# Ichoran/dbce-video-cpp

Measured on AMD Instinct MI355X. Metric: frames/s + raw-pixel GB/s, 4096x3072 U8 encode+decode round-trip, higher is better.
Workload: dtype u8

## Files before the change

### dbde-video-cpp_amd/csrc/dbde_kernels.hip

```cpp
#include "dbde_kernels.h"

#include "dbde_bits.h"
#include "dbde_device.h"


namespace dbde {

#ifndef DBDE_DIAG_LATE
#define DBDE_DIAG_LATE 34
#endif
#ifdef DBDE_DIAG
#define SF_DECL uint64_t sfd[10] = {0, 0, 0, 0, 0, 0, 0, 0, 0, 0}
#define SF_MARK(i) do { if (threadIdx.x == 0) sfd[i] = wall_clock64(); } while (0)
#define SF_DRAIN() asm volatile("s_waitcnt vmcnt(0) lgkmcnt(0)" ::: "memory")
#define SF_FLUSH(diag, last)                                                                          \
    do {                                                                                              \
        if (threadIdx.x == 0 && (diag)) {                                                             \
            atomicMax(&(diag)[0], ~(unsigned long long)sfd[0]);                                       \
            for (int i_ = 1; i_ < 10; i_++) atomicAdd(&(diag)[i_], (unsigned long long)sfd[i_]);      \
            atomicAdd(&(diag)[10], 1ull);                                                             \
            atomicMax(&(diag)[11], (unsigned long long)sfd[last]);                                    \
            atomicMax(&(diag)[12], (unsigned long long)sfd[0]);                                       \
            atomicAdd(&(diag)[13], (unsigned long long)sfd[0]);                                       \
        }                                                                                             \
// ... 1463 lines not shown
    const uint32_t seg = (cpf + blockDim.x - 1u) / blockDim.x;
    const uint32_t k0 = (uint32_t)tid * seg;
    uint32_t local = 0;
    for (uint32_t k = k0; k < k0 + seg && k < cpf; k++) local += s_sum[k];
    uint32_t incl = local;
#pragma unroll
    for (int o = 1; o < 64; o <<= 1) {
        uint32_t n = __shfl_up(incl, o, 64);
        if (lane >= o) incl += n;
    }
    if (lane == 63) s_part[wave] = incl;
    __syncthreads();
    uint32_t base = 0, total = 0;
    for (int k = 0; k < (int)(blockDim.x >> 6); k++) {
        const uint32_t v = s_part[k];
        if (k < wave) base += v;
        total += v;
    }
    uint32_t run = base + incl - local;
    uint32_t *co = p.chunk_off + (size_t)f * (cpf + 1u);
    for (uint32_t k = k0; k < k0 + seg && k < cpf; k++) {
        co[k] = run;
        run += s_sum[k];
    }
    if (tid == 0) co[cpf] = total;

    if (tid == 0) {
        bool ok = in_range;
        uint32_t field = 0;
        uint64_t index = 0, elapsed = 0, consumed = 20;
        if (in_extent(off, 20, p.stream_bytes)) {
            field = load_u32_bytes(fb);
            index = load_u64_bytes(fb + 4);
            elapsed = f64_to_u64_x86(__longlong_as_double((long long)load_u64_bytes(fb + 12)));
        }
        if (ok) {
            const int32_t nb = (int32_t)load_u32_bytes(fb + 20);
            const int32_t nm = (int32_t)load_u32_bytes(fb + 24 + T);
            const int32_t n64 = (int32_t)load_u32_bytes(fb + 28 + meta_t);
            ok = nb == (int32_t)T && nm == (int32_t)(T * p.min_bytes) && n64 == (int32_t)total && !(s_flags & 1u);
            if (ok && !in_extent(off, need + 8ull * total, p.stream_bytes)) ok = false;
            if (ok) consumed = need + 8ull * total;
        }
        p.frame_ok[f] = ok ? 1u : 0u;
        if (p.results) {
            FrameResultDev *r = reinterpret_cast<FrameResultDev *>(p.results) + f;
            r->u64s = (field == 2u && ok) ? 2u : 0xFFFFFFFFu;
            r->pad_ = 0;
            r->index = index;
            r->elapsed_ns = elapsed;
            r->consumed = consumed;
        }
    }
}

__global__ __launch_bounds__(256) void decode_index_split_kernel(IdxParams p) {
    __shared__ uint32_t s_part[4];
    __shared__ uint32_t s_last;

    const uint32_t f = blockIdx.x / p.split, piece = blockIdx.x - f * p.split;
    const int tid = threadIdx.x, lane = tid & 63, wave = tid >> 6;
    const uint32_t T = p.T, cpf = p.chunks_per_frame;
    const uint64_t off = p.frame_offsets[f];
    const uint64_t meta_t = (1ull + p.min_bytes) * T;
    const uint64_t need = 32ull + meta_t;
    const bool in_range = in_extent(off, need, p.stream_bytes);
    const uint8_t *fb = p.stream + off;
    uint32_t *co = p.chunk_off + (size_t)f * (cpf + 1u);

    const uint32_t per = (cpf + p.split - 1u) / p.split;
    const uint32_t k_begin = piece * per, k_end = k_begin + per < cpf ? k_begin + per : cpf;
    uint32_t bad = 0;
    for (uint32_t k = k_begin + (uint32_t)wave; k < k_end; k += 4u) {
        uint32_t sum = 0;
        if (in_range) {
            const uint8_t *darr = fb + 24;
            const uint32_t c_lo = dec_chunk_begin(p.geom, k), c_hi = dec_chunk_begin(p.geom, k + 1u);
#pragma unroll
            for (uint32_t j = 0; j < 8u; j += 4u) {
                const uint32_t q = c_lo + (uint32_t)lane * 8u + j;
                if (q < c_hi) {
                    uint32_t x;
                    __builtin_memcpy(&x, darr + q, 4);
                    const uint32_t keep = c_hi - q;
                    if (keep < 4u) x &= 0xFFFFFFFFu >> (8u * (4u - keep));
                    bad |= depth_bytes_bad(x, p.min_bytes);
                    sum += __builtin_amdgcn_sad_u8(x, 0u, 0u);
                }
            }
        }
        const uint32_t tot = wave_scan_incl(sum);
        if (lane == 63) __hip_atomic_store(&co[k], tot, __ATOMIC_RELAXED, __HIP_MEMORY_SCOPE_AGENT);
    }
    if (__any((int)(bad != 0u)) && lane == 0) atomicOr(&p.frame_flag[f], 1u);

    asm volatile("s_waitcnt vmcnt(0)" ::: "memory");
    __syncthreads();
    if (tid == 0) s_last = atomicAdd(&p.frame_ctr[f], 1u) == p.split - 1u ? 1u : 0u;
    __syncthreads();
    if (!s_last) return;

    const uint32_t seg = (cpf + 255u) / 256u;
    const uint32_t k0 = (uint32_t)tid * seg;
    uint32_t local = 0;
    for (uint32_t k = k0; k < k0 + seg && k < cpf; k++)
        local += __hip_atomic_load(&co[k], __ATOMIC_RELAXED, __HIP_MEMORY_SCOPE_AGENT);
    const uint32_t incl = wave_scan_incl(local);
    if (lane == 63) s_part[wave] = incl;
    __syncthreads();
    uint32_t base = 0, total = 0;
#pragma unroll
    for (int k = 0; k < 4; k++) {
        const uint32_t v = s_part[k];
        base += k < wave ? v : 0u;
        total += v;
    }
    uint32_t run = base + incl - local;
    for (uint32_t k = k0; k < k0 + seg && k < cpf; k++) {
        const uint32_t v = __hip_atomic_load(&co[k], __ATOMIC_RELAXED, __HIP_MEMORY_SCOPE_AGENT);
        co[k] = run;
        run += v;
    }
    if (tid == 0) {
        co[cpf] = total;
        const uint32_t flags = __hip_atomic_load(&p.frame_flag[f], __ATOMIC_RELAXED, __HIP_MEMORY_SCOPE_AGENT);
        p.frame_flag[f] = 0;
        p.frame_ctr[f] = 0;
        bool ok = in_range;
        uint32_t field = 0;
        uint64_t index = 0, elapsed = 0, consumed = 20;
        if (in_extent(off, 20, p.stream_bytes)) {
            field = load_u32_bytes(fb);
            index = load_u64_bytes(fb + 4);
            elapsed = f64_to_u64_x86(__longlong_as_double((long long)load_u64_bytes(fb + 12)));
        }
        if (ok) {
            const int32_t nb = (int32_t)load_u32_bytes(fb + 20);
            const int32_t nm = (int32_t)load_u32_bytes(fb + 24 + T);
            const int32_t n64 = (int32_t)load_u32_bytes(fb + 28 + meta_t);
            ok = nb == (int32_t)T && nm == (int32_t)(T * p.min_bytes) && n64 == (int32_t)total && !(flags & 1u);
            if (ok && !in_extent(off, need + 8ull * total, p.stream_bytes)) ok = false;
            if (ok) consumed = need + 8ull * total;
        }
        p.frame_ok[f] = ok ? 1u : 0u;
        if (p.results) {
            FrameResultDev *r = reinterpret_cast<FrameResultDev *>(p.results) + f;
            r->u64s = (field == 2u && ok) ? 2u : 0xFFFFFFFFu;
            r->pad_ = 0;
            r->index = index;
            r->elapsed_ns = elapsed;
            r->consumed = consumed;
        }
    }
}

hipError_t launch_decode_index(const IdxParams &p, int n_frames, hipStream_t s) {
    const size_t lds = (size_t)p.chunks_per_frame * sizeof(uint32_t);
    if (lds > 48 * 1024) {
        hipError_t e = hipFuncSetAttribute(reinterpret_cast<const void *>(decode_index_kernel),
                                           hipFuncAttributeMaxDynamicSharedMemorySize, (int)lds);
        if (e != hipSuccess) return e;
    }
    if (p.split > 1u) {
        hipLaunchKernelGGL(decode_index_split_kernel, dim3((uint32_t)n_frames * p.split), dim3(256), 0, s, p);
        return hipGetLastError();
    }
    const uint32_t pieces = (p.T + 15u) / 16u + 1u;
    uint32_t threads = (pieces + 63u) / 64u * 64u;
    threads = threads < 64u ? 64u : (threads > 1024u ? 1024u : threads);
    hipLaunchKernelGGL(decode_index_kernel, dim3(n_frames), dim3(threads), lds, s, p);
    return hipGetLastError();
}

__device__ __forceinline__ uint32_t swz_byte16(uint32_t A) { return A ^ ((A >> 4) & 0xF0u); }

__device__ __forceinline__ void put_byte1(uint32_t &x, uint32_t sh, uint32_t g) {
    asm("v_lshrrev_b32_sdwa %0, %1, %2 dst_sel:BYTE_1 dst_unused:UNUSED_PRESERVE src0_sel:DWORD src1_sel:DWORD" : "+v"(x) : "v"(sh), "v"(g));
}
__device__ __forceinline__ void put_byte2(uint32_t &x, uint32_t sh, uint32_t g) {
    asm("v_lshrrev_b32_sdwa %0, %1, %2 dst_sel:BYTE_2 dst_unused:UNUSED_PRESERVE src0_sel:DWORD src1_sel:DWORD" : "+v"(x) : "v"(sh), "v"(g));
}
__device__ __forceinline__ void put_byte3(uint32_t &x, uint32_t sh, uint32_t g) {
    asm("v_lshrrev_b32_sdwa %0, %1, %2 dst_sel:BYTE_3 dst_unused:UNUSED_PRESERVE src0_sel:DWORD src1_sel:DWORD" : "+v"(x) : "v"(sh), "v"(g));
}

template <bool SWZ>
__device__ __forceinline__ void unpack_tile_from_lds(const uint8_t *s_img, uint32_t byte_base, uint32_t d,
                                                     uint32_t mn, uint32_t (&v)[16]) {
    const uint32_t mn4 = mn * 0x01010101u;
    const bool d8 = d >= 8u;
    uint32_t a = byte_base;
    const uint32_t md = ((1u << d) - 1u) * 0x01010101u;
    const uint32_t md7 = md & 0x7F7F7F7Fu, mdh = md & 0x80808080u;
    const uint32_t mnlo = mn4 & 0x7F7F7F7Fu, mnhi = mn4 & 0x80808080u;
    const uint32_t d2 = 2u * d, d3 = 3u * d;
#pragma unroll
    for (int r = 0; r < 8; r++) {
        uint32_t t0, t1, t2;
        if (SWZ) {
            const uint32_t A0 = a & ~7u;
            const uint2 lo = *reinterpret_cast<const uint2 *>(s_img + swz_byte16(A0));
            const uint2 hi = *reinterpret_cast<const uint2 *>(s_img + swz_byte16(A0 + 8u));
            const bool up = (a & 4u) != 0u;
            t0 = up ? lo.y : lo.x; t1 = up ? hi.x : lo.y; t2 = up ? hi.y : hi.x;
        } else {
            const uint32_t *q = reinterpret_cast<const uint32_t *>(s_img + (a & ~3u));
            t0 = q[0]; t1 = q[1]; t2 = q[2];
        }
        const uint32_t r_lo = __builtin_amdgcn_alignbyte(t1, t0, a);
        const uint32_t r_hi = __builtin_amdgcn_alignbyte(t2, t1, a);
        const uint32_t g_hi = d8 ? r_hi : __builtin_amdgcn_alignbit(r_hi, r_lo, 4u * d);
        uint32_t x = r_lo, y = g_hi;
        put_byte1(x, d, r_lo); put_byte2(x, d2, r_lo); put_byte3(x, d3, r_lo);
        put_byte1(y, d, g_hi); put_byte2(y, d2, g_hi); put_byte3(y, d3, g_hi);
        v[2 * r] = (((x & md7) + mnlo) ^ (x & mdh)) ^ mnhi;
        v[2 * r + 1] = (((y & md7) + mnlo) ^ (y & mdh)) ^ mnhi;
        a += d;
    }
}

__device__ __forceinline__ void unpack_tile_d8_from_lds(const uint8_t *s_img, uint32_t byte_base, uint32_t mn,
                                                        uint32_t (&v)[16]) {
    const uint32_t mn4 = mn * 0x01010101u;
#pragma unroll
    for (int r = 0; r < 8; r++) {
        const uint2 q = *reinterpret_cast<const uint2 *>(s_img + swz_byte16(byte_base + 8u * (uint32_t)r));
        v[2 * r] = add_bytes(q.x, mn4);
        v[2 * r + 1] = add_bytes(q.y, mn4);
    }
}

constexpr uint32_t kXcdRun = 16;
__device__ __forceinline__ uint32_t xcd_local_chunk(uint32_t b, uint32_t n_chunks) {
    constexpr uint32_t kGroup = 8u * kXcdRun;
    const uint32_t grp = b / kGroup, rem = b % kGroup;
    if ((grp + 1u) * kGroup > n_chunks) return b;
    return grp * kGroup + (rem & 7u) * kXcdRun + (rem >> 3);
}

template <int THREADS = 256>
struct DecLds {
    static constexpr int kThreads = THREADS;
    static constexpr int kWaves = THREADS / 64;
    static constexpr uint32_t kSlots = THREADS == 256 ? 2128u : 1600u;
    static constexpr int kPieces = (kSlots + kThreads - 1) / kThreads;
};

__device__ __forceinline__ void lds_store_u64_any(uint8_t *s_base, uint32_t byte_addr, uint32_t lo, uint32_t hi) {
    const uint64_t v = ((uint64_t)hi << 32) | lo;
    const uint32_t a = (uint32_t)(uintptr_t)(__attribute__((address_space(3))) uint8_t *)s_base + byte_addr;
    asm volatile("ds_write_b64 %0, %1" ::"v"(a), "v"(v) : "memory");
}
__device__ __forceinline__ void lds_store_bytes(uint8_t *s_px, uint32_t a, uint64_t v, uint32_t n) {
    if (n & 4u) { __builtin_memcpy(s_px + a, &v, 4); a += 4u; v >>= 32; }
    if (n & 2u) { s_px[a] = (uint8_t)v; s_px[a + 1u] = (uint8_t)(v >> 8); a += 2u; v >>= 16; }
    if (n & 1u) s_px[a] = (uint8_t)v;
}

__device__ __forceinline__ void store_tile_generic(uint8_t *img, int W, int H, uint32_t w, uint32_t t,
                                                   const uint32_t (&v)[16]) {
    uint32_t ty = t / w, tx = t - ty * w;
    int x0 = 8 * (int)tx;
    int rm = W - x0 < 8 ? W - x0 : 8;
#pragma unroll
    for (int r = 0; r < 8; r++) {
        int yy = 8 * (int)ty + r;
        if (yy < H) {
            uint8_t *row = img + (size_t)yy * (size_t)W + x0;
            const uint64_t q = ((uint64_t)v[2 * r + 1] << 32) | v[2 * r];
            if (rm == 8) {
                store_u64_any(row, q);
            } else {
#pragma unroll
                for (int k = 0; k < 8; k++)
                    if (k < rm) row[k] = (uint8_t)(q >> (8 * k));
            }
        }
    }
}

constexpr int kImgDirect = 0, kImgLinear = 1, kImgTiles = 2;

constexpr int kIdxTable = 0, kIdxSelf = 1, kIdxFused = 2;

template <int IMG, int INDEX, int THREADS = 256>
__global__ __launch_bounds__(THREADS) void decode_kernel(DecParams p) {
    constexpr bool SELF_INDEX = INDEX == kIdxSelf;
    typedef DecLds<THREADS> G;
    __shared__ __attribute__((aligned(16))) uint64_t s_in[G::kSlots * 2];
    __shared__ uint32_t s_wave_tot[G::kWaves];
    __shared__ uint32_t s_idx[G::kWaves][4];

    const int tid = threadIdx.x, lane = tid & 63, wave = tid >> 6;
    SF_DECL;
    SF_MARK(0);
    const uint32_t c = SELF_INDEX ? blockIdx.x : xcd_local_chunk(blockIdx.x, p.n_chunks);
    const uint32_t f = c / p.chunks_per_frame;
    const uint32_t cf = c - f * p.chunks_per_frame;
    const uint64_t foff = p.frame_offsets[f];
    const uint8_t *fb = p.stream + foff;
    const uint32_t t_begin = dec_chunk_begin(p.geom, cf);
    const uint32_t n_tiles = dec_chunk_begin(p.geom, cf + 1u) - t_begin;
    uint32_t w_begin, w_end;
    if (SELF_INDEX) {
        const uint32_t T = p.T;
        const uint64_t need = 32ull + 2ull * T;
        const bool in_range = in_extent(foff, need, p.stream_bytes);
        uint32_t s_before = 0, s_mine = 0, s_all = 0, bad = 0;
        if (in_range) {
            const uint8_t *darr = fb + 24;
            const uint32_t head = (uint32_t)(reinterpret_cast<uintptr_t>(darr) & 15u);
            const uint8_t *a_lo = darr - head;
            const uint32_t npieces = (head + T + 15u) >> 4;
            const uint8_t *s_end = p.stream + p.stream_bytes;
            auto account = [&](uint32_t i, const uint4 &qv) {
                const uint32_t wv[4] = {qv.x, qv.y, qv.z, qv.w};
                const int pos0 = (int)(16u * i) - (int)head;
#pragma unroll
                for (int j = 0; j < 4; j++) {
                    const int pj = pos0 + 4 * j;
                    auto below = [&](int limit) -> uint32_t {
                        const int n = limit - pj;
                        return n >= 4 ? 0xFFFFFFFFu : (n <= 0 ? 0u : (0xFFFFFFFFu >> (8 * (4 - n))));
                    };
                    const uint32_t in = below((int)T) & ~below(0);
                    const uint32_t x = wv[j] & in;
                    bad |= (x & 0xF0F0F0F0u) | ((x + 0x77777777u) & 0x80808080u);
                    const uint32_t m0 = below((int)t_begin), m1 = below((int)(t_begin + n_tiles));
                    s_all += __builtin_amdgcn_sad_u8(x, 0u, 0u);
                    s_before += __builtin_amdgcn_sad_u8(x & m0, 0u, 0u);
                    s_mine += __builtin_amdgcn_sad_u8(x & m1 & ~m0, 0u, 0u);
                }
            };
            auto fetch = [&](uint32_t i) -> uint4 {
                if (i >= npieces) return make_uint4(0, 0, 0, 0);
                if (a_lo + 16ull * (i + 1u) <= s_end) return *reinterpret_cast<const uint4 *>(a_lo + 16ull * i);
                uint32_t wq[4] = {0, 0, 0, 0};
                for (uint32_t b = 0; b < 16u; b++) {
                    const uint8_t *src = a_lo + 16ull * i + b;
                    if (src < s_end) wq[b >> 2] |= (uint32_t)*src << (8u * (b & 3u));
                }
                return make_uint4(wq[0], wq[1], wq[2], wq[3]);
            };
            for (uint32_t i = (uint32_t)tid; i < npieces; i += 4u * (uint32_t)G::kThreads) {
                const uint4 q0 = fetch(i), q1 = fetch(i + G::kThreads), q2 = fetch(i + 2u * G::kThreads), q3 = fetch(i + 3u * G::kThreads);
                account(i, q0);
                if (i + G::kThreads < npieces) account(i + G::kThreads, q1);
                if (i + 2u * G::kThreads < npieces) account(i + 2u * G::kThreads, q2);
                if (i + 3u * G::kThreads < npieces) account(i + 3u * G::kThreads, q3);
            }
        }
        s_before = wave_sum(s_before); s_mine = wave_sum(s_mine); s_all = wave_sum(s_all);
        const bool any_bad = __any((int)(bad != 0u));
        if (lane == 0) { s_idx[wave][0] = s_before; s_idx[wave][1] = s_mine; s_idx[wave][2] = s_all; s_idx[wave][3] = any_bad ? 1u : 0u; }
        __syncthreads();
        uint32_t before = 0, mine = 0, total = 0, flag = 0;
#pragma unroll
        for (int k = 0; k < G::kWaves; k++) { before += s_idx[k][0]; mine += s_idx[k][1]; total += s_idx[k][2]; flag |= s_idx[k][3]; }
        bool okf = in_range;
        if (okf) {
            const int32_t nb = (int32_t)load_u32_bytes(fb + 20);
            const int32_t nm = (int32_t)load_u32_bytes(fb + 24 + T);
            const int32_t n64 = (int32_t)load_u32_bytes(fb + 28 + 2ull * T);
            okf = nb == (int32_t)T && nm == (int32_t)T && n64 == (int32_t)total && !flag;
            if (okf && !in_extent(foff, need + 8ull * total, p.stream_bytes)) okf = false;
        }
        if (cf == 0u && tid == 0 && p.results) {
            uint32_t field = 0;
            uint64_t index = 0, elapsed = 0;
            if (in_extent(foff, 20, p.stream_bytes)) {
                field = load_u32_bytes(fb);
                index = load_u64_bytes(fb + 4);
                elapsed = f64_to_u64_x86(__longlong_as_double((long long)load_u64_bytes(fb + 12)));
            }
            FrameResultDev *r = reinterpret_cast<FrameResultDev *>(p.results) + f;
            r->u64s = (field == 2u && okf) ? 2u : 0xFFFFFFFFu;
            r->pad_ = 0;
            r->index = index;
            r->elapsed_ns = elapsed;
            r->consumed = okf ? need + 8ull * total : 20ull;
        }
        if (!okf) return;
        w_begin = before;
        w_end = before + mine;
    } else if (INDEX == kIdxFused) {
        const uint32_t T = p.T, cpf = p.chunks_per_frame;
        const uint64_t need = 32ull + 2ull * T;
        const bool in_range = in_extent(foff, need, p.stream_bytes);
        uint32_t field = 0;
        uint64_t index = 0, elapsed = 0;
        const bool record = cf == 0u && tid == 0 && p.results;
        if (record && in_extent(foff, 20, p.stream_bytes)) {
            field = load_u32_bytes(fb);
            index = load_u64_bytes(fb + 4);
            elapsed = f64_to_u64_x86(__longlong_as_double((long long)load_u64_bytes(fb + 12)));
        }
        FrameResultDev *res = reinterpret_cast<FrameResultDev *>(p.results) + f;
        if (!in_range) {
            if (record) { res->u64s = 0xFFFFFFFFu; res->pad_ = 0; res->index = index; res->elapsed_ns = elapsed; res->consumed = 20ull; }
            return;
        }
        const int32_t nb = (int32_t)load_u32_bytes(fb + 20);
        const int32_t nm = (int32_t)load_u32_bytes(fb + 24 + T);
        const int32_t n64 = (int32_t)load_u32_bytes(fb + 28 + 2ull * T);
        const uint8_t *darr = fb + 24;
        const uint32_t te = t_begin + 2u * (uint32_t)tid;
        uint32_t dsum = 0, dbad = 0;
        if (2u * (uint32_t)tid < n_tiles) { const uint32_t d = darr[te]; dsum += d; dbad |= d > 8u ? 1u : 0u; }
        if (2u * (uint32_t)tid + 1u < n_tiles) { const uint32_t d = darr[te + 1u]; dsum += d; dbad |= d > 8u ? 1u : 0u; }
        dsum = wave_sum(dsum);
        const bool wbad = __any((int)dbad);
        if (lane == 0) { s_idx[wave][0] = dsum; s_idx[wave][1] = wbad ? 1u : 0u; }
        __syncthreads();
        SF_MARK(1);
        unsigned long long *rec = p.fuse_rec + (size_t)f * cpf;
        const unsigned long long tag = (unsigned long long)p.fuse_epoch << 32;
        if (tid == 0 && !((p.fuse_flags & 1u) && (cf & 1u))) {
            uint32_t mine = 0, mbad = 0;
#pragma unroll
            for (int k = 0; k < G::kWaves; k++) { mine += s_idx[k][0]; mbad |= s_idx[k][1]; }
            __hip_atomic_store(&rec[cf], tag | ((unsigned long long)mbad << 31) | mine, __ATOMIC_RELAXED, __HIP_MEMORY_SCOPE_AGENT);
        }
        {
            const uint64_t t_start = wall_clock64();
            uint32_t before = 0, total = 0, flag = 0;
            auto take = [&](const uint32_t base, unsigned long long w) __attribute__((always_inline)) {
                const uint32_t k = base + (uint32_t)lane;
                bool got = k >= cpf || (w >> 32) == (tag >> 32);
                for (;;) {
                    if (__all((int)got)) break;
                    if (wall_clock64() - t_start > 3000ull) {
                        uint64_t miss = __ballot((int)!got);
                        while (miss) {
                            const uint32_t kk = (uint32_t)__builtin_ctzll(miss);
                            miss &= miss - 1ull;
                            const uint32_t c_lo = dec_chunk_begin(p.geom, base + kk), c_hi = dec_chunk_begin(p.geom, base + kk + 1u);
                            uint32_t sm = 0, bd = 0;
#pragma unroll
                            for (uint32_t j = 0; j < 8u; j += 4u) {
                                const uint32_t q = c_lo + (uint32_t)lane * 8u + j;
                                if (q < c_hi) {
                                    uint32_t x;
                                    __builtin_memcpy(&x, darr + q, 4);
                                    const uint32_t keep = c_hi - q;
                                    if (keep < 4u) x &= 0xFFFFFFFFu >> (8u * (4u - keep));
                                    bd |= depth_bytes_bad(x, 1u);
                                    sm += __builtin_amdgcn_sad_u8(x, 0u, 0u);
                                }
                            }
                            sm = wave_sum(sm);
                            const bool anyb = __any((int)(bd != 0u));
                            if ((uint32_t)lane == kk) { w = tag | ((unsigned long long)(anyb ? 1u : 0u) << 31) | sm; got = true; }
                        }
                        break;
                    }
                    __builtin_amdgcn_s_sleep(1);
                    if (!got) { w = __hip_atomic_load(&rec[k], __ATOMIC_RELAXED, __HIP_MEMORY_SCOPE_AGENT); got = (w >> 32) == (tag >> 32); }
                }
                const uint32_t v = k < cpf ? (uint32_t)w & 0x7FFFFFFFu : 0u;
                total += v;
                before += k < cf ? v : 0u;
                flag |= k < cpf ? (uint32_t)(w >> 31) & 1u : 0u;
            };
            constexpr uint32_t kStride = 64u * (uint32_t)G::kWaves;
            for (uint32_t base = 64u * (uint32_t)wave; base < cpf; base += 2u * kStride) {
                const uint32_t kA = base + (uint32_t)lane, kB = kA + kStride;
                const unsigned long long wA = kA < cpf ? __hip_atomic_load(&rec[kA], __ATOMIC_RELAXED, __HIP_MEMORY_SCOPE_AGENT) : 0ull;
                const unsigned long long wB = kB < cpf ? __hip_atomic_load(&rec[kB], __ATOMIC_RELAXED, __HIP_MEMORY_SCOPE_AGENT) : 0ull;
                take(base, wA);
                if (base + kStride < cpf) take(base + kStride, wB);
            }
            before = wave_sum(before); total = wave_sum(total);
            const bool anyflag = __any((int)flag);
            if (lane == 0) { s_idx[wave][2] = before; s_idx[wave][3] = total | (anyflag ? 0x80000000u : 0u); }
        }
        SF_MARK(2);
        __syncthreads();
        uint32_t before = 0, total = 0, flag = 0;
#pragma unroll
        for (int k = 0; k < G::kWaves; k++) { before += s_idx[k][2]; total += s_idx[k][3] & 0x7FFFFFFFu; flag |= s_idx[k][3] >> 31; }
        uint32_t mine = 0;
#pragma unroll
        for (int k = 0; k < G::kWaves; k++) mine += s_idx[k][0];
        const bool okf = nb == (int32_t)T && nm == (int32_t)T && n64 == (int32_t)total && !flag &&
                         in_extent(foff, need + 8ull * total, p.stream_bytes);
        if (record) {
            res->u64s = (field == 2u && okf) ? 2u : 0xFFFFFFFFu;
            res->pad_ = 0; res->index = index; res->elapsed_ns = elapsed;
            res->consumed = okf ? need + 8ull * total : 20ull;
        }
        if (!okf) return;
        w_begin = before;
        w_end = before + mine;
        __syncthreads();
        SF_MARK(3);
    } else {
        const uint32_t ok = p.frame_ok[f];
        const uint32_t *co = p.chunk_off + (size_t)f * (p.chunks_per_frame + 1u) + cf;
        w_begin = co[0]; w_end = co[1];
        asm volatile("" :: "s"(ok), "s"(w_begin), "s"(w_end), "s"((uint32_t)foff));
        if (!ok) return;
    }

    const uint32_t t0 = t_begin + 2u * (uint32_t)tid;
    const bool hasA = 2u * (uint32_t)tid < n_tiles, hasB = 2u * (uint32_t)tid + 1u < n_tiles;
    const uint8_t *depth_arr = fb + 24;
    const uint8_t *min_arr = fb + 28 + p.T;

    const uint32_t chunk_words = w_end - w_begin;
    const uint8_t *src = fb + 32ull + 2ull * p.T + 8ull * w_begin;
    const uint32_t shift = (uint32_t)(reinterpret_cast<uintptr_t>(src) & 15u);
    const uint8_t *asrc = src - shift;
    const uint32_t n16 = (shift + 8u * chunk_words + 15u) >> 4;
    const bool swz = chunk_words == 8u * n_tiles || chunk_words == 4u * n_tiles || chunk_words == 7u * n_tiles;
    const uint32_t n16r = (n16 + 15u) & ~15u;
    const uint8_t *s_end = p.stream + p.stream_bytes;
    const uint32_t n16_dma = (asrc + 16ull * n16 <= s_end) ? n16 : n16 - 1u;
#pragma unroll
    for (int j = 0; j < G::kPieces; j++) {
        const uint32_t i = (uint32_t)tid + (uint32_t)j * G::kThreads;
        const uint32_t src_slot = swz ? swz16(i) : i;
        if (i < n16r && src_slot < n16_dma) {
            const uint32_t wave_slot0 = (uint32_t)j * G::kThreads + (uint32_t)wave * 64u;
            __builtin_amdgcn_global_load_lds(
                (const __attribute__((address_space(1))) void *)(asrc + 16ull * src_slot),
                (__attribute__((address_space(3))) void *)(&s_in[2u * wave_slot0]), 16, 0, 2 );
        }
    }
    if (n16_dma != n16 && tid < 16) {
        const uint8_t *b = asrc + 16ull * n16_dma + (uint32_t)tid;
        reinterpret_cast<uint8_t *>(s_in)[16u * (swz ? swz16(n16_dma) : n16_dma) + (uint32_t)tid] = b < s_end ? *b : (uint8_t)0;
    }
    SF_MARK(4);
    uint32_t dA = 0, dB = 0, mA = 0, mB = 0;
    if (hasB && ((reinterpret_cast<uintptr_t>(depth_arr + t0) | reinterpret_cast<uintptr_t>(min_arr + t0)) & 1u) == 0u) {
        const uint32_t d2 = *reinterpret_cast<const uint16_t *>(depth_arr + t0);
        const uint32_t m2 = *reinterpret_cast<const uint16_t *>(min_arr + t0);
        dA = d2 & 0xFFu; dB = d2 >> 8; mA = m2 & 0xFFu; mB = m2 >> 8;
    } else {
        if (hasA) { dA = depth_arr[t0]; mA = min_arr[t0]; }
        if (hasB) { dB = depth_arr[t0 + 1]; mB = min_arr[t0 + 1]; }
    }

    asm volatile("s_waitcnt vmcnt(0) lgkmcnt(0)" ::: "memory");
    SF_MARK(5);
    uint32_t chunk_total;
    const uint32_t incl = block_scan_incl<G::kWaves>(dA + dB, s_wave_tot, lane, wave, chunk_total);
    SF_MARK(6);
    const uint32_t offA = incl - (dA + dB), offB = offA + dA;

    uint32_t va[16], vb[16];
    const uint8_t *s_img = reinterpret_cast<const uint8_t *>(s_in);
    const uint32_t bA = shift + 8u * offA, bB = shift + 8u * offB;
    const bool all8 = swz && (shift & 7u) == 0u && __all((int)((dA == 8u || !hasA) && (dB == 8u || !hasB)));
    const bool flat = __all((int)((dA | dB) == 0u));
    if (flat) {
#pragma unroll
        for (int i = 0; i < 16; i++) { va[i] = mA * 0x01010101u; vb[i] = mB * 0x01010101u; }
    } else if (all8) {
        unpack_tile_d8_from_lds(s_img, bA, mA, va);
        unpack_tile_d8_from_lds(s_img, bB, mB, vb);
    } else {
        if (swz) {
            unpack_tile_from_lds<true>(s_img, bA, dA, mA, va);
            unpack_tile_from_lds<true>(s_img, bB, dB, mB, vb);
        } else {
            unpack_tile_from_lds<false>(s_img, bA, dA, mA, va);
            unpack_tile_from_lds<false>(s_img, bB, dB, mB, vb);
        }
    }

    SF_MARK(7);
    uint8_t *img = p.images + (size_t)f * p.frame_pixels;
    if (IMG == kImgDirect) {
        if (hasA) {
            const uint32_t ty = t0 / p.w, tx = t0 - ty * p.w;
            uint8_t *base = img + (size_t)(8u * tx);
#pragma unroll
            for (int r = 0; r < 8; r++) {
                const int yy = 8 * (int)ty + r;
                if (yy < p.H) {
                    u32x4_t o;
                    o[0] = va[2 * r]; o[1] = va[2 * r + 1]; o[2] = vb[2 * r]; o[3] = vb[2 * r + 1];
                    __builtin_nontemporal_store(o, reinterpret_cast<u32x4_t *>(base + (size_t)yy * (size_t)p.W));
                }
            }
        }
        SF_MARK(8);
        SF_DRAIN();
        SF_MARK(9);
        if (INDEX == kIdxFused) SF_FLUSH(p.diag, 9);
        return;
    }

    if (IMG == kImgTiles) {
        if (hasA) store_tile_generic(img, p.W, p.H, p.w, t0, va);
        if (hasB) store_tile_generic(img, p.W, p.H, p.w, t0 + 1u, vb);
        return;
    }

    const bool whole_rows = p.geom.pieces == 1u;
    const uint32_t ty0 = whole_rows ? t_begin / p.w : cf / p.geom.pieces;
    const uint32_t tx0 = whole_rows ? 0u : (cf - ty0 * p.geom.pieces) * kChunkTiles;
    const uint32_t wspan = whole_rows ? p.w : n_tiles;
    const uint32_t Wu = (uint32_t)p.W, y0 = 8u * ty0;
    const uint32_t tile_rows = whole_rows ? n_tiles / p.w : 1u;
    const uint32_t y_end = y0 + 8u * tile_rows < (uint32_t)p.H ? y0 + 8u * tile_rows : (uint32_t)p.H;
    const uint32_t x_valid = Wu - 8u * tx0 < 8u * wspan ? Wu - 8u * tx0 : 8u * wspan;
    uint8_t *g_first = img + (size_t)y0 * (size_t)p.W + (size_t)(8u * tx0);
    const uint32_t g7 = (uint32_t)(reinterpret_cast<uintptr_t>(g_first) & 127u);
    uint8_t *s_px = reinterpret_cast<uint8_t *>(s_in);
    const bool a8 = ((g7 | Wu) & 7u) == 0u;
    if (!a8 && !whole_rows) {
        if (hasA) store_tile_generic(img, p.W, p.H, p.w, t0, va);
        if (hasB) store_tile_generic(img, p.W, p.H, p.w, t0 + 1u, vb);
        return;
    }
    if (whole_rows && ((uint32_t)(reinterpret_cast<uintptr_t>(img) & 15u) | (Wu & 15u)) == 0u && chunk_words != 8u * n_tiles) {
        if (hasA) {
            const uint32_t iD = 2u * (uint32_t)tid, rowD = iD / wspan, colD = iD - rowD * wspan;
            uint8_t *base = img + (size_t)(8u * colD);
#pragma unroll
            for (int r = 0; r < 8; r++) {
                const uint32_t yy = y0 + 8u * rowD + (uint32_t)r;
                if (yy < (uint32_t)p.H) {
                    u32x4_t o;
                    o[0] = va[2 * r]; o[1] = va[2 * r + 1]; o[2] = vb[2 * r]; o[3] = vb[2 * r + 1];
                    __builtin_nontemporal_store(o, reinterpret_cast<u32x4_t *>(base + (size_t)yy * (size_t)p.W));
                }
            }
        }
        return;
    }
    __syncthreads();
    const uint32_t iA = 2u * (uint32_t)tid;
    const uint32_t rowA = iA / wspan, colA = iA - rowA * wspan;
    const uint32_t rowB = colA + 1u == wspan ? rowA + 1u : rowA, colB = colA + 1u == wspan ? 0u : colA + 1u;
    const uint32_t nA = 8u * colA + 8u <= x_valid ? 8u : x_valid - 8u * colA;
    const uint32_t nB = 8u * colB + 8u <= x_valid ? 8u : x_valid - 8u * colB;
    const bool all_rows = y0 + 8u * tile_rows <= (uint32_t)p.H;
    const bool plain = all_rows && __all((int)((!hasA || nA == 8u) && (!hasB || nB == 8u)));
    if (a8) {
        const uint32_t l_pitch = 8u * kChunkTiles + 128u;
        const uint32_t aA = whole_rows ? g7 + 8u * rowA * Wu + 8u * colA : 8u * colA;
        const uint32_t aB = whole_rows ? g7 + 8u * rowB * Wu + 8u * colB : 8u * colB;
        auto row_term = [&](uint32_t r) -> uint32_t {
            return whole_rows ? r * Wu : ((g7 + r * Wu) & 127u) + r * l_pitch;
        };
        if (plain) {
            if (hasA) {
#pragma unroll
                for (int r = 0; r < 8; r++) lds_store_u64_any(s_px, aA + row_term((uint32_t)r), va[2 * r], va[2 * r + 1]);
            }
            if (hasB) {
#pragma unroll
                for (int r = 0; r < 8; r++) lds_store_u64_any(s_px, aB + row_term((uint32_t)r), vb[2 * r], vb[2 * r + 1]);
            }
        } else {
#pragma unroll
            for (int r = 0; r < 8; r++) {
                const uint32_t rt = row_term((uint32_t)r);
                if (hasA && y0 + 8u * rowA + (uint32_t)r < y_end) {
                    if (nA == 8u) lds_store_u64_any(s_px, aA + rt, va[2 * r], va[2 * r + 1]);
                    else lds_store_bytes(s_px, aA + rt, ((uint64_t)va[2 * r + 1] << 32) | va[2 * r], nA);
                }
                if (hasB && y0 + 8u * rowB + (uint32_t)r < y_end) {
                    if (nB == 8u) lds_store_u64_any(s_px, aB + rt, vb[2 * r], vb[2 * r + 1]);
                    else lds_store_bytes(s_px, aB + rt, ((uint64_t)vb[2 * r + 1] << 32) | vb[2 * r], nB);
                }
            }
        }
        asm volatile("s_waitcnt lgkmcnt(0)" ::: "memory");
        __syncthreads();
        const uint32_t n_ranges = whole_rows ? 1u : y_end - y0;
        for (uint32_t s = 0; s < n_ranges; s++) {
            uint8_t *g0 = g_first + (size_t)s * Wu;
            const uint32_t bytes = whole_rows ? (y_end - y0) * Wu : x_valid;
            const uint32_t head = (uint32_t)(reinterpret_cast<uintptr_t>(g0) & 127u);
            uint8_t *a0 = g0 - head;
            const uint8_t *l0 = s_px + (whole_rows ? 0u : s * l_pitch);
            const uint32_t n_blocks = (head + bytes + 15u) >> 4;
            for (uint32_t j = (uint32_t)tid; j < n_blocks; j += (uint32_t)G::kThreads) {
                if (16u * j + 16u <= head || 16u * j >= head + bytes) continue;
                if (16u * j >= head && 16u * j + 16u <= head + bytes) {
                    const u32x4_t q = *reinterpret_cast<const u32x4_t *>(l0 + 16u * j);
                    __builtin_nontemporal_store(q, reinterpret_cast<u32x4_t *>(a0 + 16ull * j));
                } else {
#pragma unroll
                    for (uint32_t b = 0; b < 16u; b++) {
                        const uint32_t o = 16u * j + b;
                        if (o >= head && o < head + bytes) a0[o] = l0[o];
                    }
                }
            }
        }
        return;
    }
    const uint32_t P = 8u * wspan + 16u;
    const uint32_t aA = 8u * rowA * P + 8u * colA, aB = 8u * rowB * P + 8u * colB;
    if (hasA) {
#pragma unroll
        for (int r = 0; r < 8; r++) lds_store_u64_any(s_px, aA + (uint32_t)r * P, va[2 * r], va[2 * r + 1]);
    }
    if (hasB) {
#pragma unroll
        for (int r = 0; r < 8; r++) lds_store_u64_any(s_px, aB + (uint32_t)r * P, vb[2 * r], vb[2 * r + 1]);
    }
    asm volatile("s_waitcnt lgkmcnt(0)" ::: "memory");
    __syncthreads();
    if (hasA && colA <= 1u) {
#pragma unroll
        for (int r = 0; r < 8; r++) {
            const uint32_t ry = 8u * rowA + (uint32_t)r;
            if (ry != 0u) lds_store_u64_any(s_px, (ry - 1u) * P + Wu + 8u * colA, va[2 * r], va[2 * r + 1]);
        }
    }
    if (hasB && colB <= 1u) {
#pragma unroll
        for (int r = 0; r < 8; r++) {
            const uint32_t ry = 8u * rowB + (uint32_t)r;
            if (ry != 0u) lds_store_u64_any(s_px, (ry - 1u) * P + Wu + 8u * colB, vb[2 * r], vb[2 * r + 1]);
        }
    }
    asm volatile("s_waitcnt lgkmcnt(0)" ::: "memory");
    __syncthreads();
    {
        const uint32_t bytes = (y_end - y0) * Wu;
        uint8_t *a0 = g_first - g7;
        const uint32_t n_blocks = (g7 + bytes + 15u) >> 4;
        const uint32_t lds0 = (uint32_t)(uintptr_t)(__attribute__((address_space(3))) const uint8_t *)s_px;
        const uint32_t last_n = (g7 + bytes) & 15u;
        for (uint32_t j0 = (uint32_t)tid; j0 < n_blocks; j0 += 4u * (uint32_t)G::kThreads) {
            uint64_t d01[4], d23[4];
            uint32_t d4[4], a[4];
            bool live[4];
#pragma unroll
            for (uint32_t k = 0; k < 4u; k++) {
                const uint32_t j = j0 + k * (uint32_t)G::kThreads;
                live[k] = j < n_blocks && 16u * j + 16u > g7;
                const uint32_t o = live[k] && 16u * j > g7 ? 16u * j - g7 : 0u;
                uint32_t col;
                const uint32_t row = div_magic(o, Wu, p.magic_W, col);
                a[k] = lds0 + row * P + col;
                const uint32_t a4 = a[k] & ~3u;
                asm volatile("ds_read2_b32 %0, %3 offset1:1\n\tds_read2_b32 %1, %3 offset0:2 offset1:3\n\tds_read_b32 %2, %3 offset:16"
                             : "=&v"(d01[k]), "=&v"(d23[k]), "=&v"(d4[k]) : "v"(a4) : "memory");
            }
            asm volatile("s_waitcnt lgkmcnt(0)" : "+v"(d01[0]), "+v"(d23[0]), "+v"(d4[0]), "+v"(d01[1]), "+v"(d23[1]), "+v"(d4[1]),
                         "+v"(d01[2]), "+v"(d23[2]), "+v"(d4[2]), "+v"(d01[3]), "+v"(d23[3]), "+v"(d4[3]) :: "memory");
#pragma unroll
            for (uint32_t k = 0; k < 4u; k++) {
                const uint32_t j = j0 + k * (uint32_t)G::kThreads;
                const uint32_t w0 = (uint32_t)d01[k], w1 = (uint32_t)(d01[k] >> 32), w2 = (uint32_t)d23[k], w3 = (uint32_t)(d23[k] >> 32);
                u32x4_t q;
                q[0] = __builtin_amdgcn_alignbyte(w1, w0, a[k]);
                q[1] = __builtin_amdgcn_alignbyte(w2, w1, a[k]);
                q[2] = __builtin_amdgcn_alignbyte(w3, w2, a[k]);
                q[3] = __builtin_amdgcn_alignbyte(d4[k], w3, a[k]);
                if (!live[k]) continue;
                const bool first = 16u * j < g7, last = 16u * j + 16u > g7 + bytes;
                if (!first && !last) {
                    __builtin_nontemporal_store(q, reinterpret_cast<u32x4_t *>(a0 + 16ull * j));
                } else {
                    uint8_t *dst = first ? g_first : a0 + 16ull * j;
                    uint32_t n = first ? 16u - (g7 & 15u) : last_n;
                    if (first && last) n = bytes;
                    uint64_t lo = ((uint64_t)q[1] << 32) | q[0], hi = ((uint64_t)q[3] << 32) | q[2];
                    if (n & 8u) { store_u64_any(dst, lo); dst += 8; lo = hi; }
                    if (n & 4u) { const uint32_t v = (uint32_t)lo; __builtin_memcpy(dst, &v, 4); dst += 4; lo >>= 32; }
                    if (n & 2u) { const uint16_t v = (uint16_t)lo; __builtin_memcpy(dst, &v, 2); dst += 2; lo >>= 16; }
                    if (n & 1u) *dst = (uint8_t)lo;
                }
            }
        }
    }
}

struct MidMeta {
    uint32_t d, mn;
    uint32_t nb, nm, n64;
};

#ifndef DBDE_MID_WAVES
#define DBDE_MID_WAVES 6
#endif
template <int THREADS, bool STAGED>
__global__ __launch_bounds__(THREADS, THREADS == 1024 ? 4 : DBDE_MID_WAVES) void decode_mid_kernel(DecParams p) {
    constexpr int NW = THREADS / 64;
    __shared__ uint32_t s_tot[2][NW];
    __shared__ uint32_t s_incl[2][THREADS];
    constexpr uint32_t kMidSlot = 80u;
    __shared__ __attribute__((aligned(16))) uint8_t s_lds[THREADS * kMidSlot];
    __shared__ uint32_t s_ok[THREADS];
    __shared__ uint32_t s_bad[2];
    const uint32_t tid = threadIdx.x, lane = tid & 63u, wave = tid >> 6;
    const uint32_t T = p.T, fpw = (uint32_t)THREADS / T;
    const uint32_t fl = tid / T, t = tid - fl * T;
    const uint32_t n_frames = p.n_chunks;
    const uint32_t n_groups = (n_frames + fpw - 1u) / fpw, G = gridDim.x;
    const bool slot = fl < fpw;
    const uint32_t first = slot ? fl * T : 0u;
    const uint64_t need = 32ull + 2ull * T;
    const uint8_t *s_end = p.stream + p.stream_bytes;
    const uint32_t ty = t / p.w, tx = t - ty * p.w;
    const uint32_t Wu = (uint32_t)p.W, x0 = 8u * tx;
    const uint32_t rm = Wu - x0 < 8u ? Wu - x0 : 8u;
    const uint32_t rv = (uint32_t)p.H - 8u * ty < 8u ? (uint32_t)p.H - 8u * ty : 8u;
    const uint32_t tile_off = 8u * ty * Wu + x0;
    const bool want_results = p.results != nullptr;

    auto is_active = [&](uint32_t g) -> bool { return slot && g < n_groups && g * fpw + fl < n_frames; };
    auto get_foff = [&](uint32_t g) -> uint64_t { return is_active(g) ? p.frame_offsets[g * fpw + fl] : 0ull; };
    auto get_meta = [&](uint32_t g, uint64_t foff) -> MidMeta {
        MidMeta m;
        m.d = 0; m.mn = 0; m.nb = 0; m.nm = 0; m.n64 = 0;
        const bool active = is_active(g);
        const uint8_t *fb = p.stream + foff;
        if (active && in_extent(foff, need, p.stream_bytes)) {
            m.d = fb[24u + t]; m.mn = fb[28u + T + t];
            __builtin_memcpy(&m.nb, fb + 20, 4); __builtin_memcpy(&m.nm, fb + 24 + T, 4); __builtin_memcpy(&m.n64, fb + 28 + 2ull * T, 4);
        }
        return m;
    };

    if (STAGED && tid == 0u) { s_bad[0] = 0u; s_bad[1] = 0u; }
    uint32_t g = blockIdx.x;
    uint64_t foff_cur = get_foff(g), foff_nxt = get_foff(g + G);
    auto settle = [&](const MidMeta &x, uint32_t &dm, uint32_t &n64x) {
        dm = x.d | (x.mn << 8);
        n64x = ((int32_t)x.nb == (int32_t)T && (int32_t)x.nm == (int32_t)T) ? x.n64 : 0xFFFFFFFFu;
    };
    uint32_t dm, n64x;
    settle(get_meta(g, foff_cur), dm, n64x);
    for (uint32_t par = 0; g < n_groups; g += G, par ^= 1u) {
        MidMeta m_nxt = get_meta(g + G, foff_nxt);
        uint64_t foff_nn = get_foff(g + 2u * G);
        const bool active = is_active(g);
        const uint32_t f = g * fpw + fl;
// ... 741 lines not shown
```

### profiles/rekey.py

```python
#!/usr/bin/env python3
import hashlib
import json
import os
import re
import subprocess
import sys
import tempfile

HERE = os.path.dirname(os.path.abspath(__file__))
ROOT = os.path.dirname(HERE)
RECORDED = ("encode_kernelI", "decode_kernelI")


def bodies(path):
    out = {}
    for m in re.finditer(r"^(_ZN\w+):[^\n]*\n(.*?)\n\.Lfunc_end", open(path).read(), re.S | re.M):
        out[m.group(1)] = [re.sub(r"\.L\w+|_ZN\w+", "X", ln.strip()) for ln in m.group(2).splitlines()
                           if ln.strip() and not ln.strip().startswith((";", "."))]
    return out


def isa_sha(b):
    h = hashlib.sha256()
    for k in sorted(b):
        if any(r in k for r in RECORDED):
            h.update(k.encode())
            h.update("\n".join(b[k]).encode())
    return h.hexdigest()[:16]


def main():
    tf = os.path.join(HERE, "hbm_traffic.json")
    rec = json.load(open(tf))
    rev = sys.argv[1] if len(sys.argv) > 1 else rec.get("revision")
    if not rev:
        sys.exit("rekey: the record names no revision and none was given")
    sys.path.insert(0, ROOT)
    import bench
    now = bench.kernels_fingerprint()
    if rec.get("kernels_sha") == now:
        print(f"rekey: the record already belongs to these sources ({now})")
        return
    with tempfile.TemporaryDirectory() as tmp:
        subprocess.run(f"git -C {ROOT} archive {rev} dbde-video-cpp_amd/csrc include | tar -x -C {tmp}", shell=True, check=True)
        subprocess.run(["make", "-s", "-C", f"{tmp}/dbde-video-cpp_amd/csrc", "asm"], check=True, capture_output=True)
        subprocess.run(["make", "-s", "-C", f"{ROOT}/dbde-video-cpp_amd/csrc", "asm"], check=True, capture_output=True)
        old = bodies(f"{tmp}/dbde-video-cpp_amd/csrc/dbde_kernels.s")
        new = bodies(f"{ROOT}/dbde-video-cpp_amd/csrc/dbde_kernels.s")
    bad = []
    for k, v in old.items():
        if not any(r in k for r in RECORDED):
            continue
        if k not in new:
            bad.append(f"gone  {k}")
        elif new[k] != v:
            bad.append(f"DIFF  {k}: {len(v)} -> {len(new[k])} instructions")
    if bad:
        print("\n".join(bad))
        sys.exit(f"rekey: REFUSED -- {len(bad)} recorded kernel(s) differ from revision {rev}: the traffic record does not "
                 "describe these sources; take a new PMC pass (profiles/run_profile.sh)")
    rec["kernels_sha"] = now
    rec["revision"] = subprocess.run(["git", "-C", ROOT, "rev-parse", "--short", rev], capture_output=True, text=True, check=True).stdout.strip()
    rec["isa_sha"] = isa_sha(new)
    rec["rekeyed"] = "instruction streams of every recorded kernel identical to the pass's revision (profiles/rekey.py)"
    json.dump(rec, open(tf, "w"), indent=1)
    print(f"rekey: ok -- {sum(any(r in k for r in RECORDED) for k in old)} recorded kernel instances identical; "
          f"kernels_sha {now}, revision {rec['revision']}, isa_sha {rec['isa_sha']}")


if __name__ == "__main__":
    main()
```

### profiles/summarize.py

```python
#!/usr/bin/env python3
import csv
import glob
import json
import os
import sys
from collections import defaultdict


def read_csvs(pattern):
    rows = []
    for f in glob.glob(pattern, recursive=True):
        with open(f) as fh:
            rows += list(csv.DictReader(fh))
    return rows


def main():
    d = sys.argv[1].rstrip("/")
    tag = os.path.basename(d).replace("prof_", "")
    content = "_".join(tag.split("_")[-2:])
    out = []
    kt = read_csvs(os.path.join(d, "kt", "**", "*kernel_trace.csv"))
    dur = defaultdict(list)
    for r in kt:
        dur[r["Kernel_Name"]].append(int(r["End_Timestamp"]) - int(r["Start_Timestamp"]))
    out.append("== kernel trace (rocprofv3 --kernel-trace): name, calls, avg us, min us, max us, total us, "
               "avg us of the timed steps (the first 2 dispatches = bench.py's warm-up dropped; '-' below 6 calls)")
    start = defaultdict(list)
    for r in kt:
        start[r["Kernel_Name"]].append((int(r["Start_Timestamp"]), int(r["End_Timestamp"]) - int(r["Start_Timestamp"])))
    for k, v in sorted(dur.items(), key=lambda kv: -sum(kv[1])):
        timed = [x[1] for x in sorted(start[k])[2:]] if len(v) >= 6 else []
        steady = f"{sum(timed)/len(timed)/1e3:10.2f}" if timed else "         -"
        out.append(f"{k[:90]:90s} {len(v):6d} {sum(v)/len(v)/1e3:10.2f} {min(v)/1e3:10.2f} {max(v)/1e3:10.2f} {sum(v)/1e3:12.1f} {steady}")
    traffic = {}
    for sub in ("fetch", "write", "sq"):
        rows = read_csvs(os.path.join(d, sub, "**", "*counter_collection.csv"))
        acc = defaultdict(lambda: defaultdict(list))
        for r in rows:
            acc[r["Kernel_Name"]][r["Counter_Name"]].append(float(r["Counter_Value"]))
        out.append(f"== counters ({sub}): kernel, counter, avg per dispatch, dispatches")
        for k in acc:
            for c, v in acc[k].items():
                avg = sum(v) / len(v)
                out.append(f"{k[:70]:70s} {c:24s} {avg:18.1f} {len(v):6d}")
                if c in ("FETCH_SIZE", "WRITE_SIZE") and ("dbde::encode_kernel" in k or "dbde::decode_kernel" in k):
                    name = "dbde::encode_kernel" if "encode_kernel" in k else "dbde::decode_kernel"
                    traffic.setdefault(name, {})[c] = avg
    for name, t in traffic.items():
        if "FETCH_SIZE" in t and "WRITE_SIZE" in t:
            rd, wr = 2 * t["FETCH_SIZE"] * 1024, t["WRITE_SIZE"] * 1024
            out.append(f"== HBM traffic per launch {name}: read {rd/1e6:.1f} MB (2 x FETCH_SIZE KiB), "
                       f"write {wr/1e6:.1f} MB, total {(rd+wr)/1e6:.1f} MB")
            t["bytes"] = rd + wr
    here = os.path.dirname(os.path.abspath(__file__))
    with open(os.path.join(here, f"{tag}_summary.txt"), "w") as f:
        f.write("\n".join(out) + "\n")
    tf = os.path.join(here, "hbm_traffic.json")
    cur = json.load(open(tf)) if os.path.exists(tf) else {}
    cur[content] = {k: int(v["bytes"]) for k, v in traffic.items() if "bytes" in v}
    line = os.path.join(d, "bench_line.json")
    if os.path.exists(line):
        try:
            cur[content]["frames_per_launch"] = json.load(open(line))["config"]["frames_per_step_per_gpu"]
        except Exception:
            pass
    sys.path.insert(0, os.path.dirname(here))
    import bench
    cur["kernels_sha"] = bench.kernels_fingerprint()
    cur["tag"] = tag.split("_")[0]
    try:
        import subprocess
        root = os.path.dirname(here)
        rev = subprocess.run(["git", "-C", root, "rev-parse", "--short", "HEAD"], capture_output=True, text=True).stdout.strip()
        dirty = subprocess.run(["git", "-C", root, "status", "--porcelain", "dbde-video-cpp_amd/csrc"], capture_output=True, text=True).stdout.strip()
        if rev:
            cur["revision"] = rev + ("+dirty" if dirty else "")
    except Exception:
        pass
    cur.pop("rekeyed", None)
    cur.pop("isa_sha", None)
    json.dump(cur, open(tf, "w"), indent=1)
    print("\n".join(out))


if __name__ == "__main__":
    main()
```

Measured before the change: 119,000.

## Issue fused-index decode DMA before frame validation and reuse prefetched depth/min bytes

In the fused-index decode path, each thread now loads its depth and min bytes at the start and reuses them later instead of reloading them after the index phase. The frame acceptance check and its trailing barrier are moved after the LDS DMA issue, so payload loads start while validation finishes. Rejected frames drain outstanding loads and return. The DMA length is clamped to the stream extent when tile depths are valid. The profiling scripts also gain ISA hashing and exemption options for rekeying.

```diff
diff --git a/dbde-video-cpp_amd/csrc/dbde_kernels.hip b/dbde-video-cpp_amd/csrc/dbde_kernels.hip
--- a/dbde-video-cpp_amd/csrc/dbde_kernels.hip
+++ b/dbde-video-cpp_amd/csrc/dbde_kernels.hip
@@ -1789,6 +1789,8 @@
     const uint32_t t_begin = dec_chunk_begin(p.geom, cf);
     const uint32_t n_tiles = dec_chunk_begin(p.geom, cf + 1u) - t_begin;
     uint32_t w_begin, w_end;
+    bool accepted = true, fits = true;
+    uint32_t fdA = 0, fdB = 0, fmA = 0, fmB = 0;
     if (SELF_INDEX) {
         const uint32_t T = p.T;
         const uint64_t need = 32ull + 2ull * T;
@@ -1887,27 +1889,31 @@
             if (record) { res->u64s = 0xFFFFFFFFu; res->pad_ = 0; res->index = index; res->elapsed_ns = elapsed; res->consumed = 20ull; }
             return;
         }
+        const uint8_t *darr = fb + 24, *marr = fb + 28 + T;
+        const uint32_t te = t_begin + 2u * (uint32_t)tid;
+        if (2u * (uint32_t)tid + 1u < n_tiles && ((reinterpret_cast<uintptr_t>(darr + te) | reinterpret_cast<uintptr_t>(marr + te)) & 1u) == 0u) {
+            const uint32_t d2 = *reinterpret_cast<const uint16_t *>(darr + te);
+            const uint32_t m2 = *reinterpret_cast<const uint16_t *>(marr + te);
+            fdA = d2 & 0xFFu; fdB = d2 >> 8; fmA = m2 & 0xFFu; fmB = m2 >> 8;
+        } else {
+            if (2u * (uint32_t)tid < n_tiles) { fdA = darr[te]; fmA = marr[te]; }
+            if (2u * (uint32_t)tid + 1u < n_tiles) { fdB = darr[te + 1u]; fmB = marr[te + 1u]; }
+        }
         const int32_t nb = (int32_t)load_u32_bytes(fb + 20);
         const int32_t nm = (int32_t)load_u32_bytes(fb + 24 + T);
         const int32_t n64 = (int32_t)load_u32_bytes(fb + 28 + 2ull * T);
-        const uint8_t *darr = fb + 24;
-        const uint32_t te = t_begin + 2u * (uint32_t)tid;
-        uint32_t dsum = 0, dbad = 0;
-        if (2u * (uint32_t)tid < n_tiles) { const uint32_t d = darr[te]; dsum += d; dbad |= d > 8u ? 1u : 0u; }
-        if (2u * (uint32_t)tid + 1u < n_tiles) { const uint32_t d = darr[te + 1u]; dsum += d; dbad |= d > 8u ? 1u : 0u; }
-        dsum = wave_sum(dsum);
-        const bool wbad = __any((int)dbad);
+        const uint32_t dsum = wave_sum(fdA + fdB);
+        const bool wbad = __any((int)(fdA > 8u || fdB > 8u));
         if (lane == 0) { s_idx[wave][0] = dsum; s_idx[wave][1] = wbad ? 1u : 0u; }
         __syncthreads();
         SF_MARK(1);
+        uint32_t mine = 0, mbad = 0;
+#pragma unroll
+        for (int k = 0; k < G::kWaves; k++) { mine += s_idx[k][0]; mbad |= s_idx[k][1]; }
         unsigned long long *rec = p.fuse_rec + (size_t)f * cpf;
         const unsigned long long tag = (unsigned long long)p.fuse_epoch << 32;
-        if (tid == 0 && !((p.fuse_flags & 1u) && (cf & 1u))) {
-            uint32_t mine = 0, mbad = 0;
-#pragma unroll
-            for (int k = 0; k < G::kWaves; k++) { mine += s_idx[k][0]; mbad |= s_idx[k][1]; }
+        if (tid == 0 && !((p.fuse_flags & 1u) && (cf & 1u)))
             __hip_atomic_store(&rec[cf], tag | ((unsigned long long)mbad << 31) | mine, __ATOMIC_RELAXED, __HIP_MEMORY_SCOPE_AGENT);
-        }
         {
             const uint64_t t_start = wall_clock64();
             uint32_t before = 0, total = 0, flag = 0;
@@ -1966,21 +1972,16 @@
         uint32_t before = 0, total = 0, flag = 0;
 #pragma unroll
         for (int k = 0; k < G::kWaves; k++) { before += s_idx[k][2]; total += s_idx[k][3] & 0x7FFFFFFFu; flag |= s_idx[k][3] >> 31; }
-        uint32_t mine = 0;
-#pragma unroll
-        for (int k = 0; k < G::kWaves; k++) mine += s_idx[k][0];
-        const bool okf = nb == (int32_t)T && nm == (int32_t)T && n64 == (int32_t)total && !flag &&
-                         in_extent(foff, need + 8ull * total, p.stream_bytes);
-        if (record) {
-            res->u64s = (field == 2u && okf) ? 2u : 0xFFFFFFFFu;
-            res->pad_ = 0; res->index = index; res->elapsed_ns = elapsed;
-            res->consumed = okf ? need + 8ull * total : 20ull;
-        }
-        if (!okf) return;
         w_begin = before;
         w_end = before + mine;
-        __syncthreads();
-        SF_MARK(3);
+        fits = mbad == 0u;
+        accepted = nb == (int32_t)T && nm == (int32_t)T && n64 == (int32_t)total && !flag &&
+                   in_extent(foff, need + 8ull * total, p.stream_bytes);
+        if (record) {
+            res->u64s = (field == 2u && accepted) ? 2u : 0xFFFFFFFFu;
+            res->pad_ = 0; res->index = index; res->elapsed_ns = elapsed;
+            res->consumed = accepted ? need + 8ull * total : 20ull;
+        }
     } else {
         const uint32_t ok = p.frame_ok[f];
         const uint32_t *co = p.chunk_off + (size_t)f * (p.chunks_per_frame + 1u) + cf;
@@ -2002,7 +2003,14 @@
     const bool swz = chunk_words == 8u * n_tiles || chunk_words == 4u * n_tiles || chunk_words == 7u * n_tiles;
     const uint32_t n16r = (n16 + 15u) & ~15u;
     const uint8_t *s_end = p.stream + p.stream_bytes;
-    const uint32_t n16_dma = (asrc + 16ull * n16 <= s_end) ? n16 : n16 - 1u;
+    uint32_t n16_dma;
+    if (INDEX == kIdxFused) {
+        const uintptr_t a = reinterpret_cast<uintptr_t>(asrc), e = reinterpret_cast<uintptr_t>(s_end);
+        const uint64_t room = fits && a < e ? (uint64_t)(e - a) >> 4 : 0ull;
+        n16_dma = room < (uint64_t)n16 ? (uint32_t)room : n16;
+    } else {
+        n16_dma = (asrc + 16ull * n16 <= s_end) ? n16 : n16 - 1u;
+    }
 #pragma unroll
     for (int j = 0; j < G::kPieces; j++) {
         const uint32_t i = (uint32_t)tid + (uint32_t)j * G::kThreads;
@@ -2014,13 +2022,20 @@
                 (__attribute__((address_space(3))) void *)(&s_in[2u * wave_slot0]), 16, 0, 2 );
         }
     }
-    if (n16_dma != n16 && tid < 16) {
+    if (n16_dma != n16 && tid < 16 && (INDEX != kIdxFused || fits)) {
         const uint8_t *b = asrc + 16ull * n16_dma + (uint32_t)tid;
         reinterpret_cast<uint8_t *>(s_in)[16u * (swz ? swz16(n16_dma) : n16_dma) + (uint32_t)tid] = b < s_end ? *b : (uint8_t)0;
     }
     SF_MARK(4);
+    if (INDEX == kIdxFused && !accepted) {
+        asm volatile("s_waitcnt vmcnt(0) lgkmcnt(0)" ::: "memory");
+        return;
+    }
+    if (INDEX == kIdxFused) SF_MARK(3);
     uint32_t dA = 0, dB = 0, mA = 0, mB = 0;
-    if (hasB && ((reinterpret_cast<uintptr_t>(depth_arr + t0) | reinterpret_cast<uintptr_t>(min_arr + t0)) & 1u) == 0u) {
+    if (INDEX == kIdxFused) {
+        dA = fdA; dB = fdB; mA = fmA; mB = fmB;
+    } else if (hasB && ((reinterpret_cast<uintptr_t>(depth_arr + t0) | reinterpret_cast<uintptr_t>(min_arr + t0)) & 1u) == 0u) {
         const uint32_t d2 = *reinterpret_cast<const uint16_t *>(depth_arr + t0);
         const uint32_t m2 = *reinterpret_cast<const uint16_t *>(min_arr + t0);
         dA = d2 & 0xFFu; dB = d2 >> 8; mA = m2 & 0xFFu; mB = m2 >> 8;
diff --git a/profiles/rekey.py b/profiles/rekey.py
--- a/profiles/rekey.py
+++ b/profiles/rekey.py
@@ -29,16 +29,36 @@
     return h.hexdigest()[:16]
 
 
+def parse_args(argv):
+    rev, pattern, reason = None, None, None
+    it = iter(argv)
+    for a in it:
+        if a == "--exempt":
+            pattern = next(it, None)
+        elif a == "--reason":
+            reason = next(it, None)
+        elif a.startswith("-") or rev is not None:
+            sys.exit(f"rekey: unknown argument {a!r}")
+        else:
+            rev = a
+    if (pattern is None) != (reason is None) or (pattern is not None and not (pattern and reason.strip())):
+        sys.exit("rekey: --exempt REGEX and --reason TEXT go together, neither may be empty")
+    return rev, pattern, reason
+
+
 def main():
     tf = os.path.join(HERE, "hbm_traffic.json")
     rec = json.load(open(tf))
-    rev = sys.argv[1] if len(sys.argv) > 1 else rec.get("revision")
+    rev, pattern, reason = parse_args(sys.argv[1:])
+    rev = rev or rec.get("revision")
     if not rev:
         sys.exit("rekey: the record names no revision and none was given")
+    if rev.endswith("+dirty"):
+        sys.exit(f"rekey: the pass was taken on uncommitted sources ({rev}): name the revision that holds them")
     sys.path.insert(0, ROOT)
     import bench
     now = bench.kernels_fingerprint()
-    if rec.get("kernels_sha") == now:
+    if rec.get("kernels_sha") == now and rec.get("isa_sha"):
         print(f"rekey: the record already belongs to these sources ({now})")
         return
     with tempfile.TemporaryDirectory() as tmp:
@@ -47,24 +67,35 @@
         subprocess.run(["make", "-s", "-C", f"{ROOT}/dbde-video-cpp_amd/csrc", "asm"], check=True, capture_output=True)
         old = bodies(f"{tmp}/dbde-video-cpp_amd/csrc/dbde_kernels.s")
         new = bodies(f"{ROOT}/dbde-video-cpp_amd/csrc/dbde_kernels.s")
-    bad = []
+    bad, exempted = [], []
     for k, v in old.items():
         if not any(r in k for r in RECORDED):
             continue
-        if k not in new:
-            bad.append(f"gone  {k}")
-        elif new[k] != v:
-            bad.append(f"DIFF  {k}: {len(v)} -> {len(new[k])} instructions")
+        if k in new and new[k] == v:
+            continue
+        what = f"gone  {k}" if k not in new else f"DIFF  {k}: {len(v)} -> {len(new[k])} instructions"
+        if pattern and re.search(pattern, k):
+            exempted.append(k)
+            print("exempt " + what)
+        else:
+            bad.append(what)
     if bad:
         print("\n".join(bad))
         sys.exit(f"rekey: REFUSED -- {len(bad)} recorded kernel(s) differ from revision {rev}: the traffic record does not "
-                 "describe these sources; take a new PMC pass (profiles/run_profile.sh)")
+                 "describe these sources; take a new PMC pass (profiles/run_profile.sh, profiles/summarize.py)")
+    n = sum(any(r in k for r in RECORDED) for k in old)
     rec["kernels_sha"] = now
     rec["revision"] = subprocess.run(["git", "-C", ROOT, "rev-parse", "--short", rev], capture_output=True, text=True, check=True).stdout.strip()
     rec["isa_sha"] = isa_sha(new)
-    rec["rekeyed"] = "instruction streams of every recorded kernel identical to the pass's revision (profiles/rekey.py)"
+    if exempted:
+        rec["exempt"] = {"pattern": pattern, "reason": reason, "instances": sorted(exempted)}
+        rec["rekeyed"] = (f"instruction streams of {n - len(exempted)} of {n} recorded kernel instances identical to the pass's revision; "
+                          f"{len(exempted)} differ and are exempt, see \"exempt\" (profiles/rekey.py)")
+    else:
+        rec.pop("exempt", None)
+        rec["rekeyed"] = "instruction streams of every recorded kernel identical to the pass's revision (profiles/rekey.py)"
     json.dump(rec, open(tf, "w"), indent=1)
-    print(f"rekey: ok -- {sum(any(r in k for r in RECORDED) for k in old)} recorded kernel instances identical; "
+    print(f"rekey: ok -- {n - len(exempted)} recorded kernel instances identical, {len(exempted)} exempt; "
           f"kernels_sha {now}, revision {rec['revision']}, isa_sha {rec['isa_sha']}")
 
 
diff --git a/profiles/summarize.py b/profiles/summarize.py
--- a/profiles/summarize.py
+++ b/profiles/summarize.py
@@ -3,6 +3,7 @@
 import glob
 import json
 import os
+import subprocess
 import sys
 from collections import defaultdict
 
@@ -70,7 +71,6 @@
     cur["kernels_sha"] = bench.kernels_fingerprint()
     cur["tag"] = tag.split("_")[0]
     try:
-        import subprocess
         root = os.path.dirname(here)
         rev = subprocess.run(["git", "-C", root, "rev-parse", "--short", "HEAD"], capture_output=True, text=True).stdout.strip()
         dirty = subprocess.run(["git", "-C", root, "status", "--porcelain", "dbde-video-cpp_amd/csrc"], capture_output=True, text=True).stdout.strip()
@@ -78,8 +78,13 @@
             cur["revision"] = rev + ("+dirty" if dirty else "")
     except Exception:
         pass
+    sys.path.insert(0, here)
+    import rekey
+    csrc = os.path.join(os.path.dirname(here), "dbde-video-cpp_amd", "csrc")
+    subprocess.run(["make", "-s", "-C", csrc, "asm"], check=True, capture_output=True)
+    cur["isa_sha"] = rekey.isa_sha(rekey.bodies(os.path.join(csrc, "dbde_kernels.s")))
     cur.pop("rekeyed", None)
-    cur.pop("isa_sha", None)
+    cur.pop("exempt", None)
     json.dump(cur, open(tf, "w"), indent=1)
     print("\n".join(out))
 
```

After: 119,300 (median of 2 runs). Within noise of the previous version (+0.3%).
